# sczhou/CodeFormer

Measured on NVIDIA H100. Metric: faces_per_sec_512x512_batch32, higher is better.
Workload: dtype f32 (split-fp16 operands on tensor cores, fp32 accumulate)

## Files before the change

### codeformer_b200/csrc/conv_tc.cu

```cuda

#include <cuda.h>
#include <cuda_fp16.h>
#include <cuda_runtime.h>
#include <stdint.h>

#include <stdlib.h>

#include <atomic>
#include <mutex>

#include "conv_tc.cuh"

namespace cfb {

__global__ void tc_absmax_kernel(const float* __restrict__ w, int64_t total, unsigned* __restrict__ slot) {
  float m = 0.f;
  for (int64_t i = (int64_t)blockIdx.x * blockDim.x + threadIdx.x; i < total; i += (int64_t)gridDim.x * blockDim.x)
    m = fmaxf(m, fabsf(w[i]));
#pragma unroll
  for (int o = 16; o > 0; o >>= 1) m = fmaxf(m, __shfl_xor_sync(0xffffffffu, m, o));
  if ((threadIdx.x & 31) == 0) atomicMax(slot, __float_as_uint(m));
}

__global__ void tc_split_weights_kernel(const float* __restrict__ w, __half* __restrict__ hi, __half* __restrict__ lo,
// ... 199 lines not shown
  CFB_LAUNCH_PDL(concat_planes_kernel, dim3((unsigned)(blocks > 148 * 32 ? 148 * 32 : blocks)), dim3(256), 0, st, a, b, (__half*)planes,
                 (__half*)((char*)planes + plane), pixels, Ca, Cb);
  return 0;
}

__device__ __forceinline__ uint32_t smem_u32(const void* p) { return (uint32_t)__cvta_generic_to_shared(p); }

__device__ __forceinline__ void mbar_init(uint32_t bar, uint32_t count) {
  asm volatile("mbarrier.init.shared::cta.b64 [%0], %1;" ::"r"(bar), "r"(count) : "memory");
}
__device__ __forceinline__ void mbar_expect_tx(uint32_t bar, uint32_t bytes) {
  asm volatile("mbarrier.arrive.expect_tx.shared::cta.b64 _, [%0], %1;" ::"r"(bar), "r"(bytes) : "memory");
}
__device__ __forceinline__ void mbar_arrive(uint32_t bar) {
  asm volatile("mbarrier.arrive.shared::cta.b64 _, [%0];" ::"r"(bar) : "memory");
}
__device__ __forceinline__ void mbar_arrive_if(uint32_t bar, bool pred) {
  asm volatile("{\n\t.reg .pred p;\n\tsetp.ne.u32 p, %1, 0;\n\t@p mbarrier.arrive.shared::cta.b64 _, [%0];\n\t}"
               ::"r"(bar), "r"((uint32_t)pred) : "memory");
}
__device__ unsigned g_abort = 0;
__device__ unsigned* g_status_host = nullptr;
__device__ long long g_wait_limit = 4000000000LL;

__device__ __noinline__ void mbar_timeout() {
  atomicExch(&g_abort, 1u);
  if (g_status_host) { atomicOr_system(g_status_host, CFB_STATUS_TIMEOUT); __threadfence_system(); }
}
__device__ __noinline__ void report_overflow() {
  if (g_status_host) { atomicOr_system(g_status_host, CFB_STATUS_OVERFLOW); __threadfence_system(); }
}
template <int RELAX_NS = 0>
__device__ __forceinline__ void mbar_wait(uint32_t bar, uint32_t parity, bool& aborted) {
  uint32_t done = 0;
  uint32_t polls = 0;
  long long t0 = 0;
  while (true) {
    asm volatile(
        "{\n\t.reg .pred p;\n\t"
        "mbarrier.try_wait.parity.shared::cta.b64 p, [%1], %2, %3;\n\t"
        "selp.u32 %0, 1, 0, p;\n\t}"
        : "=r"(done)
        : "r"(bar), "r"(parity), "r"(0x989680u)
        : "memory");
    if (done) break;
    if (RELAX_NS > 0) __nanosleep(RELAX_NS);
    if ((++polls & 127u) == 0u) {
      if (*(volatile unsigned*)&g_abort) { aborted = true; break; }
      if (t0 == 0) t0 = clock64();
      else if (clock64() - t0 > *(volatile long long*)&g_wait_limit) { mbar_timeout(); aborted = true; break; }
    }
  }
  aborted = __any_sync(0xffffffffu, aborted);
}
__device__ __forceinline__ void mbar_wait(uint32_t bar, uint32_t parity) {
  uint32_t done = 0;
  const long long t0 = clock64();
  while (!done) {
    asm volatile(
        "{\n\t.reg .pred p;\n\t"
        "mbarrier.try_wait.parity.shared::cta.b64 p, [%1], %2, %3;\n\t"
        "selp.u32 %0, 1, 0, p;\n\t}"
        : "=r"(done)
        : "r"(bar), "r"(parity), "r"(0x989680u)
        : "memory");
    if (!done && clock64() - t0 > *(volatile long long*)&g_wait_limit) { mbar_timeout(); break; }
  }
}
__device__ __forceinline__ void tma_load_4d(uint32_t dst, const CUtensorMap* map, uint32_t bar, int c0, int c1, int c2, int c3) {
  asm volatile(
      "cp.async.bulk.tensor.4d.shared::cluster.global.mbarrier::complete_tx::bytes [%0], [%1, {%3, %4, %5, %6}], [%2];"
      ::"r"(dst), "l"(map), "r"(bar), "r"(c0), "r"(c1), "r"(c2), "r"(c3)
      : "memory");
}
__device__ __forceinline__ void tma_load_3d(uint32_t dst, const CUtensorMap* map, uint32_t bar, int c0, int c1, int c2) {
  asm volatile(
      "cp.async.bulk.tensor.3d.shared::cluster.global.mbarrier::complete_tx::bytes [%0], [%1, {%3, %4, %5}], [%2];"
      ::"r"(dst), "l"(map), "r"(bar), "r"(c0), "r"(c1), "r"(c2)
      : "memory");
}
__device__ __forceinline__ void tma_load_3d_hint(uint32_t dst, const CUtensorMap* map, uint32_t bar, int c0, int c1, int c2,
                                                 uint64_t policy) {
  asm volatile(
      "cp.async.bulk.tensor.3d.shared::cluster.global.mbarrier::complete_tx::bytes.L2::cache_hint [%0], [%1, {%3, %4, %5}], [%2], %6;"
      ::"r"(dst), "l"(map), "r"(bar), "r"(c0), "r"(c1), "r"(c2), "l"(policy)
      : "memory");
}
__device__ __forceinline__ uint64_t l2_evict_last_policy() {
  uint64_t pol;
  asm volatile("createpolicy.fractional.L2::evict_last.b64 %0, 1.0;" : "=l"(pol));
  return pol;
}
__device__ __forceinline__ bool elect_one() {
  uint32_t pred;
  asm volatile(
      "{\n\t.reg .b32 rx;\n\t.reg .pred px;\n\t"
      "elect.sync rx|px, 0xffffffff;\n\t"
      "selp.b32 %0, 1, 0, px;\n\t}"
      : "=r"(pred));
  return pred != 0;
}

__device__ __forceinline__ uint64_t wg_desc(uint32_t saddr, uint32_t sbo) {
  return (uint64_t)((saddr >> 4) & 0x3FFFu) | ((uint64_t)1 << 16) | ((uint64_t)((sbo >> 4) & 0x3FFFu) << 32) | ((uint64_t)1 << 62);
}
__device__ __forceinline__ void wg_fence() { asm volatile("wgmma.fence.sync.aligned;" ::: "memory"); }
// ... 152 lines not shown
  int N, Ho, Wo, Cout;
  int taps, pad, stride;
  int kw, pad_w;
  int BW, BH;
  int tiles_x, tiles_y;
  int m_tiles, n_tiles;
  int kblocks;
  int chunk;
  int a_c0, b_c0;
  int b_batched;
  int heads;
  int a_c_head, b_c_head;
  int a_img_per_head;
  int b_r_head;
  int out_per_head;
  int o_c_head;
  int up4;
  int PW, PH;
  int Hin, Win;
  int pad_mode;
  int sub;
  int out_pitch, out_c0, cout_valid;
  int res_pitch;
  const float* residual2;
  int res2_pitch;
  float post_scale;
  int fault;
  int xform;
  int a_split;
  const float* in_scale;
  const float* in_shift;
  int in_act;
  const float* bias;
  const float* residual;
  int out_act;
  const float* sft_dec;
  const float* sft_scale;
  union {
    float sft_w;
    float prelu;
  };
  const float* wscale_inv;
  float* out;
  __half* pl_hi;
  __half* pl_lo;
  float* gn_part;
  int gn_cpg;
  const float* sft_wv;
#if CFB_TC_STAMPS
  long long* dbg;
#endif
};
#if CFB_TC_STAMPS
constexpr int TC_CNT0 = 32, TC_NCNT = 8;
#define TC_STAMP(i) do { if (p.dbg != nullptr && blockIdx.x == 0) p.dbg[i] = clock64(); } while (0)
#define TC_T0(t) const long long t = clock64()
#define TC_ADD(k, t) do { if (WIDE && p.dbg != nullptr && lane == 0) \
    atomicAdd(reinterpret_cast<unsigned long long*>(p.dbg + TC_CNT0 + blockIdx.x * TC_NCNT + (k)), \
              (unsigned long long)(clock64() - (t))); } while (0)
#else
#define TC_STAMP(i) do { } while (0)
#define TC_T0(t) do { } while (0)
#define TC_ADD(k, t) do { } while (0)
#endif
#if CFB_TC_STAMPS
#define TC_VAR(v) long long v = 0
#define TC_SUM(v, t) v += clock64() - (t)
#define TC_FLUSH(k, v) do { if (WIDE && p.dbg != nullptr && lane == 0) \
    atomicAdd(reinterpret_cast<unsigned long long*>(p.dbg + TC_CNT0 + blockIdx.x * TC_NCNT + (k)), (unsigned long long)(v)); \
    v = 0; } while (0)
#else
#define TC_VAR(v) do { } while (0)
#define TC_SUM(v, t) do { } while (0)
#define TC_FLUSH(k, v) do { } while (0)
#endif
#if CFB_TC_STAMPS
__device__ __forceinline__ void tc_arrived(float v) {
  asm volatile("{\n\t.reg .pred p, q;\n\tsetp.eq.f32 p, %0, 0f00000000;\n\tvote.sync.any.pred q, p, 0xffffffff;\n\t}" ::"f"(v));
}
#endif

constexpr int XF_SKEW = 128;
constexpr int TC_A_BYTES = 128 * 128;

template <int BN>
struct TcCfg {
  static_assert(BN == 64 || BN == 128, "the wgmma engine runs 64- or 128-wide n-tiles");
  static constexpr bool WIDE = BN == 128;
  static constexpr int MMA_WARPS = WIDE ? 8 : 4;
  static constexpr int EPI_WARPS = WIDE ? 4 : 8;
  static constexpr int THREADS = WIDE ? 512 : 32 * (MMA_WARPS + 1 + EPI_WARPS);
  static constexpr int B_BYTES = BN * 128;
  static constexpr int STAGE_BYTES = 2 * TC_A_BYTES + 2 * B_BYTES;
  static constexpr int STAGES = 3;
  static constexpr int SLOT_PITCH = BN + 4;
  static constexpr int SLOT_BYTES = 128 * SLOT_PITCH * 4;
  static constexpr int SLOTS = 1;
  static constexpr int STG_BYTES = WIDE ? 0 : 8 * 4096;
  static constexpr int TAIL_BYTES = SLOT_BYTES + 1024  + 512  + STG_BYTES;
  static constexpr int SMEM_BYTES = STAGES * STAGE_BYTES + TAIL_BYTES;
  static constexpr int H_A_PLANE = 23 * 1024;
  static constexpr int H_A_SLOT = 2 * H_A_PLANE;
  static constexpr int H_A_SLOTS = 2;
  static constexpr int H_B_SLOT = 2 * B_BYTES;
  static constexpr int H_B_SLOTS = WIDE ? 2 : 4;
  static constexpr int H_SMEM_BYTES = H_A_SLOTS * H_A_SLOT + H_B_SLOTS * H_B_SLOT + TAIL_BYTES;
  static constexpr int XF_WARPS = WIDE ? 2 : 4;
  static constexpr int XF_THREADS = 32 * (MMA_WARPS + 1 + EPI_WARPS + XF_WARPS + 1);
  static_assert(!WIDE || XF_THREADS == THREADS, "the 128-wide transform variant fills the pad warps exactly");
  static constexpr int X_A_SLOTS = 2;
  static constexpr int X_A_PLANE2 = H_A_PLANE + XF_SKEW;
  static constexpr int X_B_SLOTS = H_B_SLOTS;
  static constexpr int X_SMEM_BYTES = X_A_SLOTS * H_A_SLOT + X_B_SLOTS * H_B_SLOT + TAIL_BYTES;
};

template <int BN, int CPG, bool HALO, bool XF, bool GEN = false, bool K1 = false, bool CM = false, bool SILU = false,
          bool P1 = false, bool PRELU = false>
__global__ void __launch_bounds__(XF ? TcCfg<BN>::XF_THREADS : TcCfg<BN>::THREADS, 1)
conv_tc_kernel(const __grid_constant__ CUtensorMap tmA_hi, const __grid_constant__ CUtensorMap tmA_lo,
               const __grid_constant__ CUtensorMap tmB_hi, const __grid_constant__ CUtensorMap tmB_lo, const TcParams p) {
  static_assert(!XF || HALO, "the fused operand transform exists for the halo engine only");
  static_assert(!GEN || (XF && CPG == 0), "the generalised addressing exists for the fused-transform engine only");
  static_assert(!PRELU || (BN == 64 && CPG == 0 && !K1 && !CM && !SILU && !P1 && (GEN || !HALO)),
                "the PReLU epilogue is built for the generalised and the per-tap engines");
  static_assert(!K1 || (XF && !GEN && CPG == 0), "K1 = fused transform of a 1x1 conv (patch = tile): its own instantiation");
  using Cfg = TcCfg<BN>;
  constexpr bool WIDE = Cfg::WIDE;
  static_assert(!WIDE || (HALO && !GEN && !K1 && CPG != 2), "128-wide tiles exist for the 3x3 / Upsample halo engine");
  static_assert(!CM || (BN == 64 && HALO && !GEN && !K1), "channel-major tiles exist for the 64-channel 3x3 / Upsample halo convs");
  static_assert(!P1 || (!SILU && !K1 && (GEN || WIDE || CM || !HALO)),
                "the single-pass fp16 variant is built for the generalised, 128-wide, channel-major and per-tap engines");
  constexpr int MMA_WARPS = Cfg::MMA_WARPS, EPI_WARPS = Cfg::EPI_WARPS;
  constexpr int A_SLOTS = XF ? Cfg::X_A_SLOTS : Cfg::H_A_SLOTS;
  constexpr int STAGES = Cfg::STAGES;
  constexpr int STAGE_BYTES = Cfg::STAGE_BYTES;
  const int first_tile = (int)blockIdx.x;
  const int tile_step = (int)gridDim.x;
  extern __shared__ uint8_t smem_raw[];
  uint8_t* smem = reinterpret_cast<uint8_t*>((reinterpret_cast<uintptr_t>(smem_raw) + 1023) & ~(uintptr_t)1023);
  constexpr bool HALF_B = HALO && WIDE && P1;
  constexpr int NRING = HALO ? (XF ? Cfg::X_B_SLOTS : Cfg::H_B_SLOTS) * (HALF_B ? 2 : 1) : STAGES;
  constexpr int RING_BYTES = HALO ? (HALF_B ? Cfg::B_BYTES : Cfg::H_B_SLOT) : STAGE_BYTES;
  uint8_t* ring_base = HALO ? smem + A_SLOTS * Cfg::H_A_SLOT : smem;
  float* acc_slot = reinterpret_cast<float*>(ring_base + NRING * RING_BYTES);
  uint64_t* bars = reinterpret_cast<uint64_t*>(ring_base + NRING * RING_BYTES + Cfg::SLOT_BYTES);
  uint64_t* full = bars;
  uint64_t* empty = bars + NRING;
  uint64_t* cfull = bars + 2 * NRING;
  uint64_t* cempty = bars + 2 * NRING + Cfg::SLOTS;
  uint64_t* afull = bars + 2 * NRING + 2 * Cfg::SLOTS;
  uint64_t* aempty = afull + 3;
  uint64_t* araw = aempty + 3;
  uint8_t* stage_buf = reinterpret_cast<uint8_t*>(bars) + 512;

  constexpr int NWARPS = (XF ? Cfg::XF_THREADS : Cfg::THREADS) / 32;
  const int pwarp = __shfl_sync(0xffffffffu, (int)(threadIdx.x >> 5), 0);
  const int ridx = NWARPS - 1 - pwarp;
  const int warp = pwarp < MMA_WARPS ? 1 : (ridx == 0 ? 0 : ridx + 1);
  const int lane = threadIdx.x & 31;
  bool aborted = false;
  if constexpr (WIDE) {
    if (pwarp >= MMA_WARPS) wg_regs_dec<96>();
  }
  if (threadIdx.x == 0) TC_STAMP(0);

  if (warp == 0 && lane == 0) {
    for (int a = 0; a < 3; ++a) {
      mbar_init(smem_u32(afull + a), XF ? Cfg::XF_WARPS : 1);
      mbar_init(smem_u32(aempty + a), MMA_WARPS);
      mbar_init(smem_u32(araw + a), 1);
    }
    asm volatile("prefetch.tensormap [%0];" ::"l"(&tmA_hi) : "memory");
    asm volatile("prefetch.tensormap [%0];" ::"l"(&tmA_lo) : "memory");
    asm volatile("prefetch.tensormap [%0];" ::"l"(&tmB_hi) : "memory");
    asm volatile("prefetch.tensormap [%0];" ::"l"(&tmB_lo) : "memory");
    for (int s = 0; s < NRING; ++s) { mbar_init(smem_u32(full + s), 1); mbar_init(smem_u32(empty + s), MMA_WARPS); }
    for (int a = 0; a < Cfg::SLOTS; ++a) {
      mbar_init(smem_u32(cfull + a), MMA_WARPS);
      mbar_init(smem_u32(cempty + a), EPI_WARPS);
    }
    asm volatile("fence.mbarrier_init.release.cluster;" ::: "memory");
  }
  __syncthreads();
  pdl_launch_dependents();
  pdl_wait();
  if (threadIdx.x == 0) TC_STAMP(1);

  const int total_tiles = p.m_tiles * p.n_tiles;
  const int nk = p.taps * p.kblocks;

  if (warp == 0) {
    {
      int stage = 0;
      uint32_t phase = 0;
      int aslot = 0;
      uint32_t aphase = 0;
      for (int tile = first_tile; tile < total_tiles; tile += tile_step) {
        const int mt = tile / p.n_tiles, nt = tile - mt * p.n_tiles;
        const int mtl = p.up4 ? (mt >> 2) : mt;
        const int par_y = p.up4 ? ((mt & 3) >> 1) : 0, par_x = p.up4 ? (mt & 1) : 0;
        const int per_img = p.tiles_x * p.tiles_y;
        const int n = mtl / per_img;
        const int rem = mtl - n * per_img;
        const int ty = rem / p.tiles_x, tx = rem - ty * p.tiles_x;
        const int y0 = ty * p.BH * p.stride, x0 = tx * p.BW * p.stride;
        if constexpr (HALO) {
          for (int kb = 0; kb < p.kblocks; ++kb) {
            if constexpr (!XF) {
              mbar_wait<500>(smem_u32(aempty + aslot), aphase ^ 1, aborted); if (aborted) goto teardown;
              if (elect_one()) {
                const uint32_t sa = smem_u32(smem + aslot * Cfg::H_A_SLOT);
                const uint32_t ab = smem_u32(afull + aslot);
                mbar_expect_tx(ab, (uint32_t)((P1 ? 1 : 2) * p.PW * p.PH * 128));
                tma_load_4d(sa, &tmA_hi, ab, kb * 64, x0 - p.pad, y0 - p.pad, n);
                if constexpr (!P1) tma_load_4d(sa + Cfg::H_A_PLANE, &tmA_lo, ab, kb * 64, x0 - p.pad, y0 - p.pad, n);
              }
              __syncwarp();
              if (++aslot == A_SLOTS) { aslot = 0; aphase ^= 1; }
            }
            for (int tap = 0; tap < p.taps; ++tap) {
              const int btap = p.up4 ? (mt & 3) * 4 + tap : tap;
              mbar_wait<500>(smem_u32(empty + stage), phase ^ 1, aborted); if (aborted) goto teardown;
              if (elect_one()) {
                if (tile == first_tile && tap == 0 && kb == 0) TC_STAMP(2);
                const uint32_t sb = smem_u32(ring_base + stage * RING_BYTES);
                const uint32_t fb = smem_u32(full + stage);
                const bool drop = p.fault && blockIdx.x == 0 && tile == first_tile && kb == 0 && tap == 0;
                mbar_expect_tx(fb, (uint32_t)(P1 ? Cfg::B_BYTES : Cfg::H_B_SLOT));
                if constexpr (WIDE && !P1) {
                  const uint64_t pol = l2_evict_last_policy();
                  if (!drop) tma_load_3d_hint(sb, &tmB_hi, fb, kb * 64, nt * BN, btap, pol);
// ... 8 lines not shown
            }
          }
        } else {
          for (int tap = 0; tap < p.taps; ++tap) {
            int r, s, btap = tap;
            if (p.up4) { r = (tap >> 1) + par_y; s = (tap & 1) + par_x; btap = (mt & 3) * 4 + tap; }
            else { r = tap / p.kw; s = tap - r * p.kw; }
            for (int kb = 0; kb < p.kblocks; ++kb) {
              mbar_wait<500>(smem_u32(empty + stage), phase ^ 1, aborted); if (aborted) goto teardown;
              if (elect_one()) {
                if (tile == first_tile && tap == 0 && kb == 0) TC_STAMP(2);
                const uint32_t sa = smem_u32(smem + stage * STAGE_BYTES);
                const int hh = p.heads > 1 ? n % p.heads : 0, nimg = p.heads > 1 ? n / p.heads : n;
                const int a_img = p.a_img_per_head ? n : nimg;
                const int ac = p.a_c0 + hh * p.a_c_head + kb * 64, bc = p.b_c0 + hh * p.b_c_head + kb * 64;
                const int brow = nt * BN + hh * p.b_r_head;
                const int b3 = p.b_batched ? nimg : btap;
                const uint32_t fb = smem_u32(full + stage);
                const bool drop = p.fault && blockIdx.x == 0 && tile == first_tile && kb == 0 && tap == 0;
                mbar_expect_tx(fb, (uint32_t)(P1 ? TC_A_BYTES + Cfg::B_BYTES : Cfg::STAGE_BYTES));
                tma_load_4d(sa, &tmA_hi, fb, ac, x0 + s - p.pad_w, y0 + r - p.pad, a_img);
                if constexpr (!P1) tma_load_4d(sa + TC_A_BYTES, &tmA_lo, fb, ac, x0 + s - p.pad_w, y0 + r - p.pad, a_img);
                if (!drop) tma_load_3d(sa + 2 * TC_A_BYTES, &tmB_hi, fb, bc, brow, b3);
                if constexpr (!P1) tma_load_3d(sa + 2 * TC_A_BYTES + Cfg::B_BYTES, &tmB_lo, fb, bc, brow, b3);
              }
              __syncwarp();
              if (++stage == STAGES) { stage = 0; phase ^= 1; }
            }
          }
        }
      }
    }
  } else if (warp == 1) {
    if constexpr (WIDE) wg_regs_inc<160>();
    TC_T0(t_mma);
    {
      constexpr bool N128 = WIDE || CM;
      constexpr int MH = N128 ? 1 : 2;
      const uint32_t a_sbo = HALO ? (uint32_t)(p.PW * 128) : 1024u;
      const uint32_t a_half = HALO ? (uint32_t)(8 * p.PW * 128) : 8192u;
      const int wq = (int)(threadIdx.x >> 5) & 3;
      const int wg = (int)(threadIdx.x >> 7);
      const uint32_t bar_id = 2u + (uint32_t)wg;
      const uint32_t slot_base = smem_u32(acc_slot);
      int stage = 0;
      uint32_t phase = 0;
      int slot = 0;
      uint32_t slot_phase = 0;
      int aslot = 0;
      uint32_t aphase = 0;
      float acc[MH][N128 ? 64 : 32];
      if constexpr (N128) {
        float run[64];
        auto hand_off = [&]() -> bool {
          TC_T0(t_h);
          mbar_wait(smem_u32(cempty + slot), slot_phase ^ 1, aborted);
          if (wg_any(aborted, bar_id)) return true;
          TC_ADD(2, t_h);
          const int row = wg * 64 + wq * 16 + (lane >> 2);
          uint32_t e0;
          asm volatile("mov.b32 %0, %1;" : "=r"(e0)
                       : "r"(slot_base + (uint32_t)(slot * Cfg::SLOT_BYTES) + (uint32_t)((row * Cfg::SLOT_PITCH + 2 * (lane & 3)) * 4)));
#pragma unroll
          for (int j = 0; j < 16; ++j) {
#pragma unroll
            for (int h8 = 0; h8 < 2; ++h8) {
              const uint32_t e = e0 + (uint32_t)((8 * h8 * Cfg::SLOT_PITCH + 8 * j) * 4);
              asm volatile("st.shared.v2.f32 [%0], {%1, %2};" ::"r"(e), "f"(run[4 * j + 2 * h8]), "f"(run[4 * j + 2 * h8 + 1])
                           : "memory");
            }
          }
          __syncwarp();
          if (lane == 0) mbar_arrive(smem_u32(cfull + slot));
          if (++slot == Cfg::SLOTS) { slot = 0; slot_phase ^= 1; }
          return false;
        };
        for (int tile = first_tile; tile < total_tiles; tile += tile_step) {
          const int par = p.up4 ? ((tile / p.n_tiles) & 3) : 0;
          const int par_y = par >> 1, par_x = par & 1;
          for (int c0 = 0; c0 < nk; c0 += p.chunk) {
            const int c1 = min(c0 + p.chunk, nk);
            uint32_t prev_empty = 0, prev_aempty = 0;
            for (int it = c0; it < c1; ++it) {
              const int kb = it / p.taps;
              const int tap = it - kb * p.taps;
              if (tap == 0) {
                TC_T0(t_a);
                mbar_wait(smem_u32(afull + aslot), aphase, aborted);
                if (wg_any(aborted, bar_id)) { wg_wait_all(); aborted = true; goto teardown; }
                TC_ADD(1, t_a);
              }
              int r = (p.taps == 9) ? tap / 3 : 0;
              int sft = (p.taps == 9) ? tap - r * 3 : 0;
              if (p.up4) { r = (tap >> 1) + par_y; sft = (tap & 1) + par_x; }
              const uint32_t a_hi0 = smem_u32(smem + aslot * Cfg::H_A_SLOT) + (uint32_t)((r * p.PW + sft) * 128) +
                                     (uint32_t)wg * a_half;
              const uint32_t a_lo0 = a_hi0 + (uint32_t)(XF ? Cfg::X_A_PLANE2 : Cfg::H_A_PLANE);
              const uint32_t bsm = smem_u32(ring_base + stage * RING_BYTES);
              TC_T0(t_b);
              mbar_wait(smem_u32(full + stage), phase, aborted);
              if (wg_any(aborted, bar_id)) { wg_wait_all(); aborted = true; goto teardown; }
              TC_ADD(0, t_b);
              wg_fence();
#pragma unroll
              for (int k = 0; k < 4; ++k) {
                const uint64_t db_hi = wg_desc(bsm + 32 * k, 1024u), db_lo = wg_desc(bsm + Cfg::B_BYTES + 32 * k, 1024u);
                const uint64_t da_hi = wg_desc(a_hi0 + 32 * k, a_sbo), da_lo = wg_desc(a_lo0 + 32 * k, a_sbo);
                if constexpr (P1 && CM) {
                  wg_mma_64x128(acc[0], db_hi, da_hi, (it == c0 && k == 0) ? 0u : 1u);
                } else if constexpr (P1) {
                  wg_mma_64x128(acc[0], da_hi, db_hi, (it == c0 && k == 0) ? 0u : 1u);
                } else if constexpr (CM) {
                  wg_mma_64x128(acc[0], db_hi, da_lo, (it == c0 && k == 0) ? 0u : 1u);
                  wg_mma_64x128(acc[0], db_lo, da_hi, 1u);
                  wg_mma_64x128(acc[0], db_hi, da_hi, 1u);
                } else {
                  wg_mma_64x128(acc[0], da_lo, db_hi, (it == c0 && k == 0) ? 0u : 1u);
                  wg_mma_64x128(acc[0], da_hi, db_lo, 1u);
                  wg_mma_64x128(acc[0], da_hi, db_hi, 1u);
                }
              }
              wg_commit();
              if constexpr (WIDE) {
                if (it == 0 && tile != first_tile) {
                  if (hand_off()) { wg_wait_all(); aborted = true; goto teardown; }
                }
              }
              wg_wait_1();
              __syncwarp();
              mbar_arrive_if(prev_empty, lane == 0 && prev_empty != 0);
              mbar_arrive_if(prev_aempty, lane == 0 && prev_aempty != 0);
              prev_empty = smem_u32(empty + stage);
              prev_aempty = tap == p.taps - 1 ? smem_u32(aempty + aslot) : 0u;
              if (++stage == NRING) { stage = 0; phase ^= 1; }
              if (tap == p.taps - 1 && ++aslot == A_SLOTS) { aslot = 0; aphase ^= 1; }
            }
            wg_wait_all();
            __syncwarp();
            mbar_arrive_if(prev_empty, lane == 0);
            mbar_arrive_if(prev_aempty, lane == 0 && prev_aempty != 0);
            if constexpr (CM) {
              mbar_wait(smem_u32(cempty + slot), slot_phase ^ 1, aborted);
              if (wg_any(aborted, bar_id)) { aborted = true; goto teardown; }
              const uint32_t st0 = slot_base + (uint32_t)(slot * Cfg::SLOT_BYTES) +
                                   (uint32_t)((2 * (lane & 3) * Cfg::SLOT_PITCH + wq * 16 + (lane >> 2)) * 4);
#pragma unroll
              for (int j = 0; j < 16; ++j) {
#pragma unroll
                for (int h8 = 0; h8 < 2; ++h8) {
#pragma unroll
                  for (int e = 0; e < 2; ++e) {
                    const uint32_t a = st0 + (uint32_t)(((8 * j + e) * Cfg::SLOT_PITCH + 8 * h8) * 4);
                    asm volatile("st.shared.f32 [%0], %1;" ::"r"(a), "f"(acc[0][4 * j + 2 * h8 + e]) : "memory");
                  }
                }
              }
              __syncwarp();
              if (lane == 0) mbar_arrive(smem_u32(cfull + slot));
              if (++slot == Cfg::SLOTS) { slot = 0; slot_phase ^= 1; }
              continue;
            }
            if constexpr (WIDE) {
#pragma unroll
              for (int i = 0; i < 64; ++i) run[i] = __fadd_rn(c0 == 0 ? 0.f : run[i], acc[0][i]);
            }
          }
        }
        if constexpr (WIDE) {
          if (first_tile < total_tiles && hand_off()) { aborted = true; goto teardown; }
          TC_ADD(3, t_mma);
        }
      } else {
      for (int tile = first_tile; tile < total_tiles; tile += tile_step) {
        const int par = p.up4 ? ((tile / p.n_tiles) & 3) : 0;
        const int par_y = par >> 1, par_x = par & 1;
        for (int it = 0; it < nk; ++it) {
          uint32_t a_hi0, a_lo0, bsm;
          int tap = 0;
          if constexpr (HALO) {
            const int kb = it / p.taps;
            tap = it - kb * p.taps;
            if (tap == 0) { mbar_wait(smem_u32(afull + aslot), aphase, aborted); if (wg_any(aborted)) { aborted = true; goto teardown; } }
            int r = (p.taps == 9) ? tap / 3 : 0;
            int sft = (p.taps == 9) ? tap - r * 3 : 0;
            if (p.up4) { r = (tap >> 1) + par_y; sft = (tap & 1) + par_x; }
            const uint32_t aoff = (uint32_t)((r * p.PW + sft) * 128);
            a_hi0 = smem_u32(smem + aslot * Cfg::H_A_SLOT) + aoff;
            a_lo0 = a_hi0 + (uint32_t)(XF ? Cfg::X_A_PLANE2 : Cfg::H_A_PLANE);
            bsm = smem_u32(ring_base + stage * RING_BYTES);
          } else {
            a_hi0 = smem_u32(smem + stage * STAGE_BYTES);
            a_lo0 = a_hi0 + TC_A_BYTES;
            bsm = a_hi0 + 2 * TC_A_BYTES;
          }
          mbar_wait(smem_u32(full + stage), phase, aborted); if (wg_any(aborted)) { aborted = true; goto teardown; }
          if (blockIdx.x == 0 && threadIdx.x == 0 && tile == first_tile && it == 0) TC_STAMP(3);
          const uint32_t first = (it % p.chunk) == 0 ? 1u : 0u;
          wg_fence();
#pragma unroll
          for (int k = 0; k < 4; ++k) {
            const uint64_t db_hi = wg_desc(bsm + 32 * k, 1024u), db_lo = wg_desc(bsm + Cfg::B_BYTES + 32 * k, 1024u);
#pragma unroll
            for (int mh = 0; mh < 2; ++mh) {
              const uint64_t da_hi = wg_desc(a_hi0 + mh * a_half + 32 * k, a_sbo), da_lo = wg_desc(a_lo0 + mh * a_half + 32 * k, a_sbo);
              if constexpr (P1) {
                wg_mma_64x64(acc[mh], da_hi, db_hi, (first && k == 0) ? 0u : 1u);
              } else {
                wg_mma_64x64(acc[mh], da_lo, db_hi, (first && k == 0) ? 0u : 1u);
                wg_mma_64x64(acc[mh], da_hi, db_lo, 1u);
                wg_mma_64x64(acc[mh], da_hi, db_hi, 1u);
              }
            }
          }
          wg_commit();
          wg_wait_all();
          __syncwarp();
          if (lane == 0) mbar_arrive(smem_u32(empty + stage));
          if (++stage == NRING) { stage = 0; phase ^= 1; }
          if constexpr (HALO) {
            if (tap == p.taps - 1) {
              if (lane == 0) mbar_arrive(smem_u32(aempty + aslot));
              if (++aslot == A_SLOTS) { aslot = 0; aphase ^= 1; }
// ... 96 lines not shown
          if (t == 0 && tile == first_tile + tile_step && kb == 0) TC_STAMP(19);
          const uint32_t base0 = smem_u32(smem + aslot * Cfg::H_A_SLOT);
          const uint32_t src_base = base0 + (pl ? (uint32_t)Cfg::X_A_PLANE2 : 0u);
          const uint32_t lo_base = base0 + (uint32_t)Cfg::X_A_PLANE2;
          if constexpr (K1) {
            if (mode == 2) xf_patch<2, RPP, NPASS1, 8, 128>(src_base, base0, lo_base, c0, j, rsub, sc, sh, border, y0, x0, Hin, Win, amax);
            else if (mode == 1) xf_patch<1, RPP, NPASS1, 8, 128>(src_base, base0, lo_base, c0, j, rsub, sc, sh, border, y0, x0, Hin, Win, amax);
            else xf_patch<0, RPP, NPASS1, 8, 128>(src_base, base0, lo_base, c0, j, rsub, sc, sh, border, y0, x0, Hin, Win, amax);
          } else {
            if (mode == 2) xf_patch<2, RPP, NPASS, XF_PW, XF_ROWS, !P1>(src_base, base0, lo_base, c0, j, rsub, sc, sh, border, y0, x0, Hin, Win, amax);
            else if (mode == 1) xf_patch<1, RPP, NPASS, XF_PW, XF_ROWS, !P1>(src_base, base0, lo_base, c0, j, rsub, sc, sh, border, y0, x0, Hin, Win, amax);
            else xf_patch<0, RPP, NPASS, XF_PW, XF_ROWS, !P1>(src_base, base0, lo_base, c0, j, rsub, sc, sh, border, y0, x0, Hin, Win, amax);
          }
          if constexpr (GEN) {
            if (p.pad_mode && border) {
              asm volatile("bar.sync 1, %0;" ::"r"(32 * XFW) : "memory");
#pragma unroll 1
              for (int r = rsub; r < XF_ROWS; r += RPP) {
                const int py = r / XF_PW, px = r - py * XF_PW;
                const int gy = y0 + py, gx = x0 + px;
                if ((unsigned)gy < (unsigned)Hin && (unsigned)gx < (unsigned)Win) continue;
                int sy = gy, sx = gx;
                if (p.pad_mode == 1) {
                  sy = sy < 0 ? -sy : (sy >= Hin ? 2 * Hin - 2 - sy : sy);
                  sx = sx < 0 ? -sx : (sx >= Win ? 2 * Win - 2 - sx : sx);
                }
                sy = min(max(sy, max(y0, 0)), min(Hin, y0 + XF_PH) - 1);
                sx = min(max(sx, max(x0, 0)), min(Win, x0 + XF_PW) - 1);
                const int rs = (sy - y0) * XF_PW + (sx - x0);
                const uint32_t hs = base0 + (uint32_t)rs * 128u, hd = base0 + (uint32_t)r * 128u;
                const uint32_t ls = lo_base + (uint32_t)rs * 128u, ld = lo_base + (uint32_t)r * 128u;
                const uint4 hv = lds128(hs + ((((uint32_t)j) ^ ((hs >> 7) & 7u)) << 4));
                if constexpr (P1) {
                  sts128(hd + ((((uint32_t)j) ^ ((hd >> 7) & 7u)) << 4), hv);
                } else {
                  const uint4 lv = lds128(ls + ((((uint32_t)j) ^ ((ls >> 7) & 7u)) << 4));
                  sts128(hd + ((((uint32_t)j) ^ ((hd >> 7) & 7u)) << 4), hv);
                  sts128(ld + ((((uint32_t)j) ^ ((ld >> 7) & 7u)) << 4), lv);
                }
              }
            }
          }
          asm volatile("fence.proxy.async.shared::cta;" ::: "memory");
          __syncwarp();
          if (lane == 0) mbar_arrive(smem_u32(afull + aslot));
          if (t == 0 && tile == first_tile && kb == 0) TC_STAMP(12);
          if (t == 0 && tile == first_tile + tile_step && kb == 0) TC_STAMP(20);
          if (++aslot == A_SLOTS) { aslot = 0; aphase ^= 1; }
        }
      }
      if (amax > 65504.f) report_overflow();
    }
  } else {
    constexpr int HC = BN * 4 / EPI_WARPS;
    const int lg = (warp - 2) & 3;
    const int half = (warp - 2) >> 2;
    const int row = lg * 32 + lane;
    const int cbase = half * HC;
    const float wsi = __ldg(p.wscale_inv);
    const int BW = HALO ? 8 : p.BW, BH = HALO ? 16 : p.BH;
    const int bw_shift = HALO ? 3 : ((BW & (BW - 1)) == 0 ? __ffs(BW) - 1 : -1);
    const int64_t SW = (int64_t)(p.up4 ? 2 : 1) * (HALO ? p.Cout : p.out_pitch), SH = SW * p.Wo;
    const int ts = p.up4 ? 2 : 1;
    const bool whole_tiles = HALO || (p.tiles_y * BH * ts == p.Ho && p.tiles_x * BW * ts == p.Wo);
    int slot = 0;
    uint32_t slot_phase = 0;
    float omax = 0.f;
    TC_T0(t_epi);
    TC_VAR(c_ld);
    TC_VAR(c_st);
    for (int tile = first_tile; tile < total_tiles; tile += tile_step) {
      const int pm = tile / p.n_tiles, nt = tile - pm * p.n_tiles;
      const int mt = pm;
      const int mtl = p.up4 ? (mt >> 2) : mt;
      const int per_img = p.tiles_x * p.tiles_y;
      const int nb = mtl / per_img;
      const int rem = mtl - nb * per_img;
      const bool hsplit = !HALO && p.heads > 1 && !p.out_per_head;
      const int n = hsplit ? nb / p.heads : nb;
      const int ty = rem / p.tiles_x, tx = rem - ty * p.tiles_x;
      const int h = bw_shift >= 0 ? (row >> bw_shift) : row / BW, w = row - h * BW;
      int oy = ty * BH + h, ox = tx * BW + w;
      if (p.up4) { oy = 2 * oy + ((mt & 3) >> 1); ox = 2 * ox + (mt & 1); }
      const int64_t pix = ((int64_t)n * p.Ho + oy) * p.Wo + ox;
      const int64_t off_tile = (((int64_t)n * p.Ho + (p.up4 ? 2 * ty * BH + ((mt & 3) >> 1) : ty * BH)) * p.Wo +
                                (p.up4 ? 2 * tx * BW + (mt & 1) : tx * BW)) * (HALO ? p.Cout : p.out_pitch);
      const int col0 = nt * BN + cbase + (hsplit ? (nb % p.heads) * p.o_c_head : 0);
      const int64_t off0 = pix * (HALO ? p.Cout : p.out_pitch) + col0;
      const bool row_in = whole_tiles || (oy < p.Ho && ox < p.Wo);
      if (!GEN && p.residual && row_in) {
#pragma unroll
        for (int j = 0; j < HC; j += 32) asm volatile("prefetch.global.L2 [%0];" ::"l"(p.residual + off0 + j));
      }
      if (p.sft_dec && row_in) {
#pragma unroll
        for (int j = 0; j < HC; j += 32) {
          asm volatile("prefetch.global.L2 [%0];" ::"l"(p.sft_dec + off0 + j));
          asm volatile("prefetch.global.L2 [%0];" ::"l"(p.sft_scale + off0 + j));
        }
      }
      float acc[WIDE ? 1 : HC];
      if constexpr (WIDE) {
        TC_T0(t_c);
        mbar_wait<250>(smem_u32(cfull + slot), slot_phase, aborted); if (aborted) goto teardown;
        TC_ADD(4, t_c);
      } else {
#pragma unroll
        for (int j = 0; j < HC; ++j) acc[j] = 0.f;
        for (int it0 = 0; it0 < nk; it0 += p.chunk) {
          mbar_wait<250>(smem_u32(cfull + slot), slot_phase, aborted); if (aborted) goto teardown;
          const uint32_t srow = smem_u32(acc_slot) + (uint32_t)(slot * Cfg::SLOT_BYTES) + (uint32_t)((row * Cfg::SLOT_PITCH + cbase) * 4);
#pragma unroll
          for (int c0 = 0; c0 < HC; c0 += 4) {
            const float4 v = lds128f(srow + (uint32_t)(c0 * 4));
            acc[c0] += v.x; acc[c0 + 1] += v.y; acc[c0 + 2] += v.z; acc[c0 + 3] += v.w;
          }
          asm volatile("" ::: "memory");
          __syncwarp();
          if (lane == 0) mbar_arrive(smem_u32(cempty + slot));
          if (++slot == Cfg::SLOTS) { slot = 0; slot_phase ^= 1; }
        }
      }
      if (warp == 2 && lane == 0 && tile == first_tile) TC_STAMP(7);
      if (warp == 2 && lane == 0 && tile == first_tile + tile_step) TC_STAMP(17);
      const uint32_t stg = smem_u32(stage_buf) + (uint32_t)(warp - 2) * 4096u;
      const uint32_t stg_w = stg + (uint32_t)lane * 128u;
      const int cch = lane & 7, rsub = lane >> 3;
      if constexpr (GEN) {
        const int Hs = p.sub ? (p.Ho >> 1) : p.Ho, Ws = p.sub ? (p.Wo >> 1) : p.Wo;
#pragma unroll
        for (int q = 0; q < HC; q += 32) {
#pragma unroll
          for (int j = 0; j < 8; ++j)
            sts128f(stg_w + (uint32_t)((j ^ (lane & 7)) << 4), acc[q + 4 * j] * wsi, acc[q + 4 * j + 1] * wsi, acc[q + 4 * j + 2] * wsi,
                    acc[q + 4 * j + 3] * wsi);
          __syncwarp();
          const int colq = col0 + q + cch * 4;
          const bool col_ok = colq < p.cout_valid;
          float4 bv = make_float4(0.f, 0.f, 0.f, 0.f);
          if (p.bias) bv = __ldg(reinterpret_cast<const float4*>(p.bias + colq));
          int64_t pixs[8];
#pragma unroll
          for (int it = 0; it < 8; ++it) {
            const int trow = lg * 32 + it * 4 + rsub;
            const int hh = trow / BW, ww = trow - hh * BW;
            int oy2 = ty * BH + hh, ox2 = tx * BW + ww;
            if (p.up4) { oy2 = 2 * oy2 + ((mt & 3) >> 1); ox2 = 2 * ox2 + (mt & 1); }
            bool ok = col_ok && n < p.N && oy2 < p.Ho && ox2 < p.Wo;
            if (p.sub) { ok = ok && (((oy2 | ox2) & 1) == 0); oy2 >>= 1; ox2 >>= 1; }
            pixs[it] = ok ? ((int64_t)n * Hs + oy2) * Ws + ox2 : (int64_t)-1;
          }
          float4 rres[8];
#pragma unroll
          for (int it = 0; it < 8; ++it)
            rres[it] = (p.residual && pixs[it] >= 0) ? __ldg(reinterpret_cast<const float4*>(p.residual + pixs[it] * p.res_pitch + colq))
                                                     : make_float4(0.f, 0.f, 0.f, 0.f);
#pragma unroll
          for (int it = 0; it < 8; ++it) {
            const int r = it * 4 + rsub;
            float4 v = lds128f(stg + (uint32_t)(r * 128 + ((cch ^ (r & 7)) << 4)));
            v.x += bv.x + rres[it].x; v.y += bv.y + rres[it].y; v.z += bv.z + rres[it].z; v.w += bv.w + rres[it].w;
            if constexpr (PRELU) {
              v.x = v.x > 0.f ? v.x : p.prelu * v.x; v.y = v.y > 0.f ? v.y : p.prelu * v.y;
              v.z = v.z > 0.f ? v.z : p.prelu * v.z; v.w = v.w > 0.f ? v.w : p.prelu * v.w;
            } else if (p.out_act == OUT_LRELU || p.out_act == OUT_RELU) {
              const float sl = p.out_act == OUT_LRELU ? 0.2f : 0.f;
              v.x = v.x > 0.f ? v.x : sl * v.x; v.y = v.y > 0.f ? v.y : sl * v.y;
              v.z = v.z > 0.f ? v.z : sl * v.z; v.w = v.w > 0.f ? v.w : sl * v.w;
            } else if (SILU) {
              v.x = tc_silu_out(v.x); v.y = tc_silu_out(v.y); v.z = tc_silu_out(v.z); v.w = tc_silu_out(v.w);
            }
            if (pixs[it] >= 0) {
              if (p.residual2) {
                const float4 r2 = __ldg(reinterpret_cast<const float4*>(p.residual2 + pixs[it] * p.res2_pitch + colq));
                v.x = fmaf(v.x, p.post_scale, r2.x); v.y = fmaf(v.y, p.post_scale, r2.y);
                v.z = fmaf(v.z, p.post_scale, r2.z); v.w = fmaf(v.w, p.post_scale, r2.w);
              }
              *reinterpret_cast<float4*>(p.out + pixs[it] * p.out_pitch + p.out_c0 + colq) = v;
            }
          }
          __syncwarp();
        }
      } else {
      const uint32_t slot_q = smem_u32(acc_slot) + (uint32_t)(slot * Cfg::SLOT_BYTES) +
                              (uint32_t)(((lg * 32 + rsub) * Cfg::SLOT_PITCH + cbase + cch * 4) * 4);
#pragma unroll
      for (int q = 0; q < HC; q += 32) {
        if constexpr (!WIDE) {
#pragma unroll
          for (int j = 0; j < 8; ++j)
            sts128f(stg_w + (uint32_t)((j ^ (lane & 7)) << 4), acc[q + 4 * j] * wsi, acc[q + 4 * j + 1] * wsi, acc[q + 4 * j + 2] * wsi,
                    acc[q + 4 * j + 3] * wsi);
          __syncwarp();
        }
        const int colq = col0 + q + cch * 4;
        float4 bv = make_float4(0.f, 0.f, 0.f, 0.f);
        if (p.bias) bv = __ldg(reinterpret_cast<const float4*>(p.bias + colq));
        constexpr int RB = (XF || WIDE) ? 4 : 8;
        float s0 = 0.f, q0 = 0.f, s1 = 0.f, q1 = 0.f, k0 = 0.f, k1 = 0.f;
#pragma unroll
        for (int ib = 0; ib < 8; ib += RB) {
        int64_t offs[RB];
        bool inside[RB];
#pragma unroll
        for (int k = 0; k < RB; ++k) {
          const int it = ib + k;
          const int trow = lg * 32 + it * 4 + rsub;
          const int hh = bw_shift >= 0 ? (trow >> bw_shift) : trow / BW, ww = trow - hh * BW;
          offs[k] = off_tile + colq + hh * SH + ww * SW;
          inside[k] = whole_tiles || ((ty * BH + hh) * ts < p.Ho && (tx * BW + ww) * ts < p.Wo);
        }
        TC_T0(t_l);
        float4 rres[RB];
#pragma unroll
        for (int k = 0; k < RB; ++k)
          rres[k] = (p.residual && inside[k]) ? __ldg(reinterpret_cast<const float4*>(p.residual + offs[k])) : make_float4(0.f, 0.f, 0.f, 0.f);
#if CFB_TC_STAMPS
        if (WIDE && p.residual) { tc_arrived(rres[RB - 1].w); TC_SUM(c_ld, t_l); }
#endif
#pragma unroll
        for (int k = 0; k < RB; ++k) {
          const int it = ib + k;
          const int r = it * 4 + rsub;
          float4 v;
          if constexpr (WIDE) {
            v = lds128f(slot_q + (uint32_t)((it * 4 * Cfg::SLOT_PITCH + q) * 4));
            v.x = __fmul_rn(v.x, wsi); v.y = __fmul_rn(v.y, wsi); v.z = __fmul_rn(v.z, wsi); v.w = __fmul_rn(v.w, wsi);
          } else {
            v = lds128f(stg + (uint32_t)(r * 128 + ((cch ^ (r & 7)) << 4)));
          }
          const int64_t off = offs[k];
          v.x += bv.x + rres[k].x; v.y += bv.y + rres[k].y; v.z += bv.z + rres[k].z; v.w += bv.w + rres[k].w;
          if constexpr (PRELU) {
            v.x = v.x > 0.f ? v.x : p.prelu * v.x; v.y = v.y > 0.f ? v.y : p.prelu * v.y;
            v.z = v.z > 0.f ? v.z : p.prelu * v.z; v.w = v.w > 0.f ? v.w : p.prelu * v.w;
          } else if (p.out_act == OUT_LRELU) {
            v.x = v.x > 0.f ? v.x : 0.2f * v.x; v.y = v.y > 0.f ? v.y : 0.2f * v.y;
            v.z = v.z > 0.f ? v.z : 0.2f * v.z; v.w = v.w > 0.f ? v.w : 0.2f * v.w;
          } else if (p.out_act == OUT_GELU) {
// ... 22 lines not shown
          TC_T0(t_st);
          const bool col_in = HALO || colq < p.cout_valid;
          if (p.out && inside[k] && col_in) *reinterpret_cast<float4*>(p.out + off) = v;
          if (p.pl_hi && inside[k]) {
            omax = fmaxf(omax, fmaxf(fmaxf(fabsf(v.x), fabsf(v.y)), fmaxf(fabsf(v.z), fabsf(v.w))));
            const __half2 h01 = __floats2half2_rn(v.x, v.y), h23 = __floats2half2_rn(v.z, v.w);
            const float2 f01 = __half22float2(h01), f23 = __half22float2(h23);
            const __half2 l01 = __floats2half2_rn(v.x - f01.x, v.y - f01.y), l23 = __floats2half2_rn(v.z - f23.x, v.w - f23.y);
            uint2 ph, pl;
            ph.x = *reinterpret_cast<const uint32_t*>(&h01); ph.y = *reinterpret_cast<const uint32_t*>(&h23);
            pl.x = *reinterpret_cast<const uint32_t*>(&l01); pl.y = *reinterpret_cast<const uint32_t*>(&l23);
            *reinterpret_cast<uint2*>(p.pl_hi + off) = ph;
            *reinterpret_cast<uint2*>(p.pl_lo + off) = pl;
          }
          TC_SUM(c_st, t_st);
          if constexpr (CPG == 2) {
            if (it == 0) { k0 = v.x; k1 = v.z; }
            const float a = v.x - k0, b = v.y - k0, c = v.z - k1, d = v.w - k1;
            s0 += a + b; q0 += fmaf(a, a, b * b);
            s1 += c + d; q1 += fmaf(c, c, d * d);
          } else if constexpr (CPG >= 4) {
            if (it == 0) k0 = v.x;
            const float a = v.x - k0, b = v.y - k0, c = v.z - k0, d = v.w - k0;
            s0 += (a + b) + (c + d);
            q0 += fmaf(a, a, b * b) + fmaf(c, c, d * d);
          }
        }
        }
        if constexpr (CPG > 0) {
          constexpr float NL = CPG == 2 ? 16.f : 32.f;
          gn_lane_moments(s0, q0, k0, NL);
          if constexpr (CPG == 2) gn_lane_moments(s1, q1, k1, NL);
          gn_merge_xor(s0, q0, 8, NL); gn_merge_xor(s0, q0, 16, 2.f * NL);
          if constexpr (CPG == 2) { gn_merge_xor(s1, q1, 8, NL); gn_merge_xor(s1, q1, 16, 2.f * NL); }
          if constexpr (CPG >= 8) gn_merge_xor(s0, q0, 1, 4.f * NL);
          if constexpr (CPG >= 16) gn_merge_xor(s0, q0, 2, 8.f * NL);
          constexpr int CL = (CPG >= 4) ? CPG / 4 : 1;
          TC_T0(t_gs);
          if (rsub == 0 && (cch & (CL - 1)) == 0) {
            float* gp = p.gn_part + ((int64_t)mt * 4 + lg) * 64;
            if constexpr (CPG == 2) {
              *reinterpret_cast<float4*>(gp + (colq / 2) * 2) = make_float4(s0, q0, s1, q1);
            } else {
              *reinterpret_cast<float2*>(gp + (colq / CPG) * 2) = make_float2(s0, q0);
            }
          }
          TC_SUM(c_st, t_gs);
        }
        __syncwarp();
      }
      }
      if constexpr (WIDE) {
        if (lane == 0) mbar_arrive(smem_u32(cempty + slot));
        if (++slot == Cfg::SLOTS) { slot = 0; slot_phase ^= 1; }
        TC_FLUSH(5, c_ld);
        TC_FLUSH(6, c_st);
      }
      if (warp == 2 && lane == 0 && tile == first_tile) TC_STAMP(16);
      if (warp == 2 && lane == 0 && tile == first_tile + tile_step) TC_STAMP(18);
    }
    if (omax > 65504.f) report_overflow();
    TC_ADD(7, t_epi);
    if (warp == 2 && lane == 0) TC_STAMP(13);
  }

teardown:
  if (aborted) {
    const long long t0 = clock64();
    while (clock64() - t0 < 400000) {}
  }
  __syncthreads();
  if (threadIdx.x == 0) TC_STAMP(8);
}

int tc_bind_status_word(unsigned* host_mapped_dev_ptr, long long wait_limit_cycles) {
  const unsigned zero = 0;
  CFB_CUDA(cudaMemcpyToSymbol(g_status_host, &host_mapped_dev_ptr, sizeof(host_mapped_dev_ptr)));
  CFB_CUDA(cudaMemcpyToSymbol(g_wait_limit, &wait_limit_cycles, sizeof(wait_limit_cycles)));
  CFB_CUDA(cudaMemcpyToSymbol(g_abort, &zero, sizeof(zero)));
  return 0;
}
static std::atomic<int> g_inject_fault{0};
static std::atomic<long long*> g_stamps{nullptr};
int tc_set_stamps(long long* dev_ptr) { g_stamps.store(dev_ptr); return 0; }
int tc_inject_fault(int kind) { g_inject_fault.store(kind); return 0; }
int tc_clear_abort() {
  const unsigned zero = 0;
  CFB_CUDA(cudaMemcpyToSymbol(g_abort, &zero, sizeof(zero)));
  return 0;
}

typedef CUresult (*EncodeTiledFn)(CUtensorMap*, CUtensorMapDataType, cuuint32_t, void*, const cuuint64_t*, const cuuint64_t*,
                                  const cuuint32_t*, const cuuint32_t*, CUtensorMapInterleave, CUtensorMapSwizzle,
                                  CUtensorMapL2promotion, CUtensorMapFloatOOBfill);

static EncodeTiledFn get_encode_fn() {
  static EncodeTiledFn fn = nullptr;
  static std::once_flag once;
  std::call_once(once, [] {
    void* p = nullptr;
    cudaDriverEntryPointQueryResult q;
    if (cudaGetDriverEntryPoint("cuTensorMapEncodeTiled", &p, cudaEnableDefault, &q) == cudaSuccess &&
        q == cudaDriverEntryPointSuccess)
      fn = (EncodeTiledFn)p;
  });
  return fn;
}

static int make_map(CUtensorMap* m, const void* base, int rank, const uint64_t* dims, const uint64_t* strides_bytes,
                    const uint32_t* box, int spatial_stride = 1, bool f32 = false) {
  EncodeTiledFn fn = get_encode_fn();
  CFB_REQUIRE(fn != nullptr, "cuTensorMapEncodeTiled is not available from the driver");
// ... 790 lines not shown
```

Baseline: 195.7.

## Split 128-wide accumulator hand-off into per-warpgroup half slots with opportunistic early handoff

```diff
diff --git a/codeformer_b200/csrc/conv_tc.cu b/codeformer_b200/csrc/conv_tc.cu
--- a/codeformer_b200/csrc/conv_tc.cu
+++ b/codeformer_b200/csrc/conv_tc.cu
@@ -275,6 +275,17 @@
     }
   }
   aborted = __any_sync(0xffffffffu, aborted);
+}
+__device__ __forceinline__ bool mbar_test(uint32_t bar, uint32_t parity) {
+  uint32_t done;
+  asm volatile(
+      "{\n\t.reg .pred p;\n\t"
+      "mbarrier.test_wait.parity.shared::cta.b64 p, [%1], %2;\n\t"
+      "selp.u32 %0, 1, 0, p;\n\t}"
+      : "=r"(done)
+      : "r"(bar), "r"(parity)
+      : "memory");
+  return done != 0;
 }
 __device__ __forceinline__ void mbar_wait(uint32_t bar, uint32_t parity) {
   uint32_t done = 0;
@@ -533,7 +544,7 @@
 #endif
 };
 #if CFB_TC_STAMPS
-constexpr int TC_CNT0 = 32, TC_NCNT = 8;
+constexpr int TC_CNT0 = 32, TC_NCNT = 9;
 #define TC_STAMP(i) do { if (p.dbg != nullptr && blockIdx.x == 0) p.dbg[i] = clock64(); } while (0)
 #define TC_T0(t) const long long t = clock64()
 #define TC_ADD(k, t) do { if (WIDE && p.dbg != nullptr && lane == 0) \
@@ -575,8 +586,10 @@
   static constexpr int STAGE_BYTES = 2 * TC_A_BYTES + 2 * B_BYTES;
   static constexpr int STAGES = 3;
   static constexpr int SLOT_PITCH = BN + 4;
-  static constexpr int SLOT_BYTES = 128 * SLOT_PITCH * 4;
+  static constexpr int SLOT_ROWS = WIDE ? 64 : 128;
+  static constexpr int SLOT_BYTES = SLOT_ROWS * SLOT_PITCH * 4;
   static constexpr int SLOTS = 1;
+  static constexpr int CBARS = WIDE ? 2 : SLOTS;
   static constexpr int STG_BYTES = WIDE ? 0 : 8 * 4096;
   static constexpr int TAIL_BYTES = SLOT_BYTES + 1024  + 512  + STG_BYTES;
   static constexpr int SMEM_BYTES = STAGES * STAGE_BYTES + TAIL_BYTES;
@@ -584,7 +597,7 @@
   static constexpr int H_A_SLOT = 2 * H_A_PLANE;
   static constexpr int H_A_SLOTS = 2;
   static constexpr int H_B_SLOT = 2 * B_BYTES;
-  static constexpr int H_B_SLOTS = WIDE ? 2 : 4;
+  static constexpr int H_B_SLOTS = WIDE ? 3 : 4;
   static constexpr int H_SMEM_BYTES = H_A_SLOTS * H_A_SLOT + H_B_SLOTS * H_B_SLOT + TAIL_BYTES;
   static constexpr int XF_WARPS = WIDE ? 2 : 4;
   static constexpr int XF_THREADS = 32 * (MMA_WARPS + 1 + EPI_WARPS + XF_WARPS + 1);
@@ -593,6 +606,8 @@
   static constexpr int X_A_PLANE2 = H_A_PLANE + XF_SKEW;
   static constexpr int X_B_SLOTS = H_B_SLOTS;
   static constexpr int X_SMEM_BYTES = X_A_SLOTS * H_A_SLOT + X_B_SLOTS * H_B_SLOT + TAIL_BYTES;
+  static_assert(!WIDE || (H_SMEM_BYTES == 227840 && X_SMEM_BYTES == 227840), "128-wide halo layout");
+  static_assert(H_SMEM_BYTES <= 232448 && X_SMEM_BYTES <= 232448, "shared memory budget");
 };
 
 template <int BN, int CPG, bool HALO, bool XF, bool GEN = false, bool K1 = false, bool CM = false, bool SILU = false,
@@ -622,14 +637,15 @@
   constexpr bool HALF_B = HALO && WIDE && P1;
   constexpr int NRING = HALO ? (XF ? Cfg::X_B_SLOTS : Cfg::H_B_SLOTS) * (HALF_B ? 2 : 1) : STAGES;
   constexpr int RING_BYTES = HALO ? (HALF_B ? Cfg::B_BYTES : Cfg::H_B_SLOT) : STAGE_BYTES;
+  static_assert((2 * NRING + 2 * Cfg::CBARS + 9) * 8 <= 512, "barriers must fit their 512-byte region");
   uint8_t* ring_base = HALO ? smem + A_SLOTS * Cfg::H_A_SLOT : smem;
   float* acc_slot = reinterpret_cast<float*>(ring_base + NRING * RING_BYTES);
   uint64_t* bars = reinterpret_cast<uint64_t*>(ring_base + NRING * RING_BYTES + Cfg::SLOT_BYTES);
   uint64_t* full = bars;
   uint64_t* empty = bars + NRING;
   uint64_t* cfull = bars + 2 * NRING;
-  uint64_t* cempty = bars + 2 * NRING + Cfg::SLOTS;
-  uint64_t* afull = bars + 2 * NRING + 2 * Cfg::SLOTS;
+  uint64_t* cempty = bars + 2 * NRING + Cfg::CBARS;
+  uint64_t* afull = bars + 2 * NRING + 2 * Cfg::CBARS;
   uint64_t* aempty = afull + 3;
   uint64_t* araw = aempty + 3;
   uint8_t* stage_buf = reinterpret_cast<uint8_t*>(bars) + 512;
@@ -656,8 +672,8 @@
     asm volatile("prefetch.tensormap [%0];" ::"l"(&tmB_hi) : "memory");
     asm volatile("prefetch.tensormap [%0];" ::"l"(&tmB_lo) : "memory");
     for (int s = 0; s < NRING; ++s) { mbar_init(smem_u32(full + s), 1); mbar_init(smem_u32(empty + s), MMA_WARPS); }
-    for (int a = 0; a < Cfg::SLOTS; ++a) {
-      mbar_init(smem_u32(cfull + a), MMA_WARPS);
+    for (int a = 0; a < Cfg::CBARS; ++a) {
+      mbar_init(smem_u32(cfull + a), WIDE ? 4 : MMA_WARPS);
       mbar_init(smem_u32(cempty + a), EPI_WARPS);
     }
     asm volatile("fence.mbarrier_init.release.cluster;" ::: "memory");
@@ -772,15 +788,17 @@
       float acc[MH][N128 ? 64 : 32];
       if constexpr (N128) {
         float run[64];
+        uint32_t ho = (uint32_t)(wg ^ 1);
+        auto ho_bar = [&]() { return slot_base + (uint32_t)(Cfg::SLOT_BYTES + (2 * NRING + Cfg::CBARS + (wg ^ 1)) * 8); };
         auto hand_off = [&]() -> bool {
           TC_T0(t_h);
-          mbar_wait(smem_u32(cempty + slot), slot_phase ^ 1, aborted);
+          mbar_wait(ho_bar(), ho & 1u, aborted);
           if (wg_any(aborted, bar_id)) return true;
-          TC_ADD(2, t_h);
-          const int row = wg * 64 + wq * 16 + (lane >> 2);
+          TC_ADD(wg ? 8 : 2, t_h);
+          const int row = wq * 16 + (lane >> 2);
           uint32_t e0;
           asm volatile("mov.b32 %0, %1;" : "=r"(e0)
-                       : "r"(slot_base + (uint32_t)(slot * Cfg::SLOT_BYTES) + (uint32_t)((row * Cfg::SLOT_PITCH + 2 * (lane & 3)) * 4)));
+                       : "r"(slot_base + (uint32_t)((row * Cfg::SLOT_PITCH + 2 * (lane & 3)) * 4)));
 #pragma unroll
           for (int j = 0; j < 16; ++j) {
 #pragma unroll
@@ -791,8 +809,8 @@
             }
           }
           __syncwarp();
-          if (lane == 0) mbar_arrive(smem_u32(cfull + slot));
-          if (++slot == Cfg::SLOTS) { slot = 0; slot_phase ^= 1; }
+          if (lane == 0) mbar_arrive(smem_u32(cfull + wg));
+          ho = (ho & 1u) ^ 1u;
           return false;
         };
         for (int tile = first_tile; tile < total_tiles; tile += tile_step) {
@@ -842,7 +860,7 @@
               }
               wg_commit();
               if constexpr (WIDE) {
-                if (it == 0 && tile != first_tile) {
+                if ((ho & 2u) && (wg == 0 || !wg_any(!mbar_test(ho_bar(), ho & 1u), bar_id))) {
                   if (hand_off()) { wg_wait_all(); aborted = true; goto teardown; }
                 }
               }
@@ -881,13 +899,17 @@
               continue;
             }
             if constexpr (WIDE) {
+              if ((ho & 2u) && hand_off()) { aborted = true; goto teardown; }
+            }
+            if constexpr (WIDE) {
 #pragma unroll
               for (int i = 0; i < 64; ++i) run[i] = __fadd_rn(c0 == 0 ? 0.f : run[i], acc[0][i]);
             }
           }
+          if constexpr (WIDE) ho |= 2u;
         }
         if constexpr (WIDE) {
-          if (first_tile < total_tiles && hand_off()) { aborted = true; goto teardown; }
+          if ((ho & 2u) && hand_off()) { aborted = true; goto teardown; }
           TC_ADD(3, t_mma);
         }
       } else {
@@ -1090,11 +1112,9 @@
       if (amax > 65504.f) report_overflow();
     }
   } else {
-    constexpr int HC = BN * 4 / EPI_WARPS;
-    const int lg = (warp - 2) & 3;
-    const int half = (warp - 2) >> 2;
-    const int row = lg * 32 + lane;
-    const int cbase = half * HC;
+    constexpr int NHALF = WIDE ? 2 : 1;
+    constexpr int HC = WIDE ? 64 : BN * 4 / EPI_WARPS;
+    const int cbase = ((warp - 2) >> (WIDE ? 1 : 2)) * HC;
     const float wsi = __ldg(p.wscale_inv);
     const int BW = HALO ? 8 : p.BW, BH = HALO ? 16 : p.BH;
     const int bw_shift = HALO ? 3 : ((BW & (BW - 1)) == 0 ? __ffs(BW) - 1 : -1);
@@ -1107,7 +1127,9 @@
     TC_T0(t_epi);
     TC_VAR(c_ld);
     TC_VAR(c_st);
-    for (int tile = first_tile; tile < total_tiles; tile += tile_step) {
+    for (int tile = first_tile, hf = 0; tile < total_tiles; hf = (hf + 1) % NHALF, tile += hf == 0 ? tile_step : 0) {
+      const int lg = WIDE ? 2 * hf + ((warp - 2) & 1) : (warp - 2) & 3;
+      const int row = lg * 32 + lane;
       const int pm = tile / p.n_tiles, nt = tile - pm * p.n_tiles;
       const int mt = pm;
       const int mtl = p.up4 ? (mt >> 2) : mt;
@@ -1156,11 +1178,11 @@
           asm volatile("" ::: "memory");
           __syncwarp();
           if (lane == 0) mbar_arrive(smem_u32(cempty + slot));
-          if (++slot == Cfg::SLOTS) { slot = 0; slot_phase ^= 1; }
+          if (++slot == Cfg::CBARS) { slot = 0; slot_phase ^= 1; }
         }
       }
-      if (warp == 2 && lane == 0 && tile == first_tile) TC_STAMP(7);
-      if (warp == 2 && lane == 0 && tile == first_tile + tile_step) TC_STAMP(17);
+      if (warp == 2 && lane == 0 && hf == 0 && tile == first_tile) TC_STAMP(7);
+      if (warp == 2 && lane == 0 && hf == 0 && tile == first_tile + tile_step) TC_STAMP(17);
       const uint32_t stg = smem_u32(stage_buf) + (uint32_t)(warp - 2) * 4096u;
       const uint32_t stg_w = stg + (uint32_t)lane * 128u;
       const int cch = lane & 7, rsub = lane >> 3;
@@ -1220,9 +1242,8 @@
           __syncwarp();
         }
       } else {
-      const uint32_t slot_q = smem_u32(acc_slot) + (uint32_t)(slot * Cfg::SLOT_BYTES) +
-                              (uint32_t)(((lg * 32 + rsub) * Cfg::SLOT_PITCH + cbase + cch * 4) * 4);
-#pragma unroll
+      const uint32_t slot_q = smem_u32(acc_slot) + (uint32_t)((((lg & 1) * 32 + rsub) * Cfg::SLOT_PITCH + cbase + cch * 4) * 4);
+#pragma unroll 1
       for (int q = 0; q < HC; q += 32) {
         if constexpr (!WIDE) {
 #pragma unroll
@@ -1351,12 +1372,12 @@
       }
       if constexpr (WIDE) {
         if (lane == 0) mbar_arrive(smem_u32(cempty + slot));
-        if (++slot == Cfg::SLOTS) { slot = 0; slot_phase ^= 1; }
+        if (++slot == Cfg::CBARS) { slot = 0; slot_phase ^= 1; }
         TC_FLUSH(5, c_ld);
         TC_FLUSH(6, c_st);
       }
-      if (warp == 2 && lane == 0 && tile == first_tile) TC_STAMP(16);
-      if (warp == 2 && lane == 0 && tile == first_tile + tile_step) TC_STAMP(18);
+      if (warp == 2 && lane == 0 && hf == NHALF - 1 && tile == first_tile) TC_STAMP(16);
+      if (warp == 2 && lane == 0 && hf == NHALF - 1 && tile == first_tile + tile_step) TC_STAMP(18);
     }
     if (omax > 65504.f) report_overflow();
     TC_ADD(7, t_epi);
```

Measured after the change: 198.7, median of 6. About the same (+1.5%).
